# ai-forever/Kandinsky-5

Measured on AMD Instinct MI355X. Metric: DiT denoising steps/sec (2B Lite, 5s 768x512 latent), higher is better.
Workload: dtype bf16

## Files before the change

include/k5.h:

```cpp
#ifndef K5_H
#define K5_H
#include <stdint.h>
#ifdef __cplusplus
extern "C" {
#endif

typedef enum {
  K5_OK = 0, K5_ERR_ARG = 1, K5_ERR_ALIGN = 2, K5_ERR_HIP = 3, K5_ERR_STATE = 4, K5_ERR_KEY = 5,
  K5_ERR_UNSUPPORTED = 6
} k5_status;
typedef enum { K5_F32 = 0, K5_BF16 = 1, K5_F16 = 2 } k5_dtype;
typedef enum { K5_EPI_BIAS = 0, K5_EPI_BIAS_M = 1, K5_EPI_GELU = 2, K5_EPI_GATE = 3, K5_EPI_F32 = 4  } k5_epilogue;

#define K5_ABI_VERSION 11
int k5_abi_version(void);
const char* k5_last_error(void);


int k5_gemm_bf16(const void* A, const void* W, const float* bias, void* C, int M, int N, int K, int lda,
                 int ldw, int ldc, int epilogue, const void* resid, int ldr, const float* gate, void* stream);
int k5_gemm_bf16_variant(const void* A, const void* W, const float* bias, void* C, int M, int N, int K, int lda, int ldw, int ldc,
                         int epilogue, const void* resid, int ldr, const float* gate, void* stream, int kernel, int token_tile);

int k5_gemm_bf16_f32out(const void* A, const void* W, float* C, int M, int N, int K, int lda, int ldw, int ldc,
                        float alpha, int causal_hw, void* stream);

int k5_causal_softmax_bf16(const float* scores, void* P, int S, int hw, int lds, int ldp, void* stream);
int k5_vae_attention512_bf16(const void* q, const void* k, const void* vt, void* o, int S, int hw, int ldqk, int ldvt, int ldo,
                             float scale, void* stream);

int k5_attention_bf16(const void* Q, const void* K, const void* Vt, void* O, int H, int q_len, int kv_len,
                      int ldq, int ldk, int ldvt, int ldo, void* stream);

int64_t k5_attention_state_size(int H, int q_len);
int k5_attention_bf16_range(const void* Q, const void* K, const void* Vt, void* O, int H, int q_len, int kv_len,
                            int ldq, int ldk, int ldvt, int ldo, float score_bound, int tile_off0, int tile_cnt,
                            int tile_skip_at, int tile_skip_n, void* state, int flags, void* stream);
// ... 245 lines not shown
```

kandinsky-5_amd/csrc/engine.hip:

```cpp
#include <math.h>
#include <stdarg.h>
#include <stdio.h>
#include <stdlib.h>
#include <string.h>

#include <map>
#include <optional>
#include <string>
#include <vector>

#include <dlfcn.h>
#include <pthread.h>
#include <rccl/rccl.h>

#include "k5_common.h"
#include "k5_kernels.h"
#include "ipc_comm.h"

static thread_local char g_err[1024] = "";
void k5_set_error(const char* fmt, ...) {
  va_list ap;
  va_start(ap, fmt);
  vsnprintf(g_err, sizeof(g_err), fmt, ap);
  va_end(ap);
// ... 274 lines not shown
  DevBuf ws_attn_bal;
  DevBuf ws_attn_stats, ws_attn_flags, ws_attn_cnt, ws_attn_part;
  long long nabla_possible = 0;
  int nabla_list_rows = 4;
  int attn_mode = 0;
  int sp_pass1_tiles = 0;
  int nabla_group_rows = 0, nabla_grp_now = 4;
  int nabla_pair_frames = 1;
  void* nabla_tap = nullptr; long long nabla_tap_cap = 0, nabla_tap_n = 0;
  int nabla_fuse_means = 1;
  DevBuf ws_nabla_kept;
  unsigned long long* h_nabla_kept = nullptr;
  long long nabla_hint_possible = 0;
  bool nabla_hint_pending = false;
  int sp_nabla_passes = 1;
  int fuse_qnorm = 0;
  int fuse_qnorm_auto = 1;
  bool fuse_now = false, leave_collect = false;
  int fuse_last = -1;
  DevBuf ws_leave_sig;
  DevBuf ws_pref_snap;
  unsigned int* h_leave_sig = nullptr;
  bool row_offsets = true;
  bool anchor = true;
  DevBuf ws_attn_anchor;
  int sp_slices = 1;
  int sp_mode = 0;
  DevBuf ws_u_send, ws_u_recv, ws_u_vsend, ws_u_vrecv, ws_u_o, ws_u_orecv, ws_u_stats;
  hipEvent_t ev_u_o = nullptr, ev_u_back = nullptr;
  DevBuf ws_u_qrecv;
// ... 291 lines not shown
  const bool vis = !strcmp(fam_attn, "attn_self");
  const bool f8_in = vis && sa_fp8_in(d, a, rows);
  const bool f8_out = vis && (d->fp8_mask & 4) && a.wo8.p && rows >= 256;
  if (h8_ready && !f8_in) { k5_set_error("internal: e4m3 activations handed to a bf16 projection"); return K5_ERR_ARG; }
  if (f8_in) {
    K5CHK(d->ws_h8.ensure((size_t)rows * D));
    if (!h8_ready) {
      Scope sc(d, s, "elementwise");
      K5CHK(k5_launch_quant_rows_fp8(h, d->ws_h8.p, nullptr, rows, D, D, D, s));
    }
    Scope sc(d, s, "gemm");
    K5CHK(k5_launch_gemm_fp8(d->ws_h8.p, a.wqk8.p, a.sqk.as<float>(), qk, rows, 2 * D, D, D, D, 2 * D, K5_EPI_BIAS, nullptr, 0, nullptr, s, a.bqk.as<float>(), 0));
    K5CHK(k5_launch_gemm_fp8(a.wv8.p, d->ws_h8.p, a.sv.as<float>(), vt, D, rows, D, D, D, ldvt, K5_EPI_BIAS, nullptr, 0, nullptr, s, a.bv.as<float>(), 1));
  } else {
    Scope sc(d, s, "gemm");
    K5CHK(k5_launch_gemm_bf16(h, a.wqk.p, a.bqk.as<float>(), qk, rows, 2 * D, D, D, D, 2 * D, K5_EPI_BIAS, nullptr, 0, nullptr, s));
    K5CHK(k5_launch_gemm_bf16(a.wv.p, h, a.bv.as<float>(), vt, D, rows, D, D, D, ldvt, K5_EPI_BIAS_M, nullptr, 0, nullptr, s));
  }
  const bool pre = vis && rows % 64 == 0;
  const bool by_data = pre && d->attn_mode == K5_ATTN_AUTO;
  SoftmaxForm sf;
  const bool fuse_q = pre && !nabla && (d->fuse_qnorm || d->fuse_now) && ((by_data && d->row_offsets) || d->attn_mode == K5_ATTN_ONLINE);
  unsigned int* leave_sig = (d->leave_collect && d->ws_leave_sig.p) ? d->ws_leave_sig.as<unsigned int>() : nullptr;
  const bool fuse_means = pre && nabla && nabla_means_fused(d, rows, 2 * H);
  const int grp = pre ? attn_group_rows(d, nabla != nullptr, false) : 4;
  if (by_data) K5CHK(ensure_attn_flags(d, s));
  const K5QueryNorm qn{a.norm.as<float>(), cosT, sinT, by_data ? d->ws_attn_cnt.as<unsigned long long>() : nullptr};
  {
    Scope sc(d, s, "elementwise");
    const int32_t hc[2] = {H, 2 * H};
    void* kc = nullptr;
    void *mq = nullptr, *mk = nullptr;
// ... 1737 lines not shown
    if (value != K5_ATTN_AUTO && value != K5_ATTN_ONLINE) { k5_set_error("attn_mode must be 0 or 1"); return K5_ERR_ARG; }
    d->attn_mode = value; return K5_OK;
  }
  if (!strcmp(name, "sp_pass1_tiles")) { if (value < 0) return K5_ERR_ARG; d->sp_pass1_tiles = value; return K5_OK; }
  if (!strcmp(name, "sp_mode")) { if (value < 0 || value > 2) return K5_ERR_ARG; d->sp_mode = value; d->sp_user_set |= 1; return K5_OK; }
  if (!strcmp(name, "sp_autotune")) { d->sp_autotune = value != 0; if (value > 1) d->sp_tuned = false; return K5_OK; }
  if (!strcmp(name, "attn_row_offsets")) { d->row_offsets = value != 0; return K5_OK; }
  if (!strcmp(name, "attn_anchor")) { d->anchor = value != 0; return K5_OK; }
  if (!strcmp(name, "attn_pref_reset")) return reset_attn_pref(d, nullptr, true);
  if (!strcmp(name, "cross_kv_batched")) { if (value != 0 && value != 1) return K5_ERR_ARG; d->cross_kv_batched = value; return K5_OK; }
  if (!strcmp(name, "nabla_fuse_means")) { if (value < 0 || value > 2) return K5_ERR_ARG; d->nabla_fuse_means = value; return K5_OK; }
  if (!strcmp(name, "fp8_fuse_ln")) { if (value != 0 && value != 1) return K5_ERR_ARG; d->fp8_fuse_ln = value; return K5_OK; }
  if (!strcmp(name, "nabla_pair_frames")) { if (value != 0 && value != 1) return K5_ERR_ARG; d->nabla_pair_frames = value; return K5_OK; }
  if (!strcmp(name, "nabla_group_rows")) { if (value != 0 && value != 1 && value != 2 && value != 4) return K5_ERR_ARG; d->nabla_group_rows = value; return K5_OK; }
  if (!strcmp(name, "sp_nabla_passes")) { if (value < 1 || value > 2) return K5_ERR_ARG; d->sp_nabla_passes = value; d->sp_user_set |= 4; return K5_OK; }
  if (!strcmp(name, "attn_fuse_qnorm")) { if (value < 0 || value > 2) return K5_ERR_ARG; d->fuse_qnorm = value; return K5_OK; }
  if (!strcmp(name, "attn_fuse_qnorm_auto")) { if (value != 0 && value != 1) return K5_ERR_ARG; d->fuse_qnorm_auto = value; return K5_OK; }
  if (!strcmp(name, "sp_slices")) {
    if (value < 1 || value > 4) return K5_ERR_ARG;
    if (value > 1 && d->comm.comm && !d->comm.can_exchange()) { k5_set_error("sp_slices > 1 needs ncclSend / ncclRecv / ncclGroup* in the RCCL library"); return K5_ERR_STATE; }
    d->sp_slices = value; d->sp_user_set |= 2; return K5_OK;
  }
  if (!strcmp(name, "emulate_world")) {
    if (!d->comm.active() || d->comm.world != 1 || value < 1) { k5_set_error("emulate_world needs a world = 1 communicator"); return K5_ERR_STATE; }
    d->sp_world = value; d->emulated = value > 1;
    if (d->emulated) fprintf(stderr, "libk5: emulate_world=%d — timing-only layout, the results of this handle are garbage\n", value);
    return K5_OK;
  }
  k5_set_error("unknown option %s", name);
  return K5_ERR_ARG;
}
extern "C" int k5_dit_get_option(k5_dit* d, const char* name, int* value) {
  if (!d || !name || !value) return K5_ERR_ARG;
  if (!strcmp(name, "attn_mode")) *value = d->attn_mode;
  else if (!strcmp(name, "sp_pass1_tiles")) *value = d->sp_pass1_tiles;
  else if (!strcmp(name, "sp_mode")) *value = d->sp_mode;
  else if (!strcmp(name, "sp_mode_used")) *value = d->sp_mode_used;
  else if (!strcmp(name, "sp_slices")) *value = d->sp_slices;
  else if (!strcmp(name, "attn_row_offsets")) *value = d->row_offsets ? 1 : 0;
  else if (!strcmp(name, "attn_anchor")) *value = d->anchor ? 1 : 0;
  else if (!strcmp(name, "attn_fuse_qnorm")) *value = d->fuse_qnorm;
  else if (!strcmp(name, "attn_fuse_qnorm_auto")) *value = d->fuse_qnorm_auto;
  else if (!strcmp(name, "attn_fuse_qnorm_used")) *value = d->fuse_last;
  else if (!strcmp(name, "sp_nabla_passes")) *value = d->sp_nabla_passes;
  else if (!strcmp(name, "sp_autotune")) *value = d->sp_autotune ? 1 : 0;
  else if (!strcmp(name, "sp_tuned")) *value = d->sp_tuned ? 1 : 0;
  else if (!strcmp(name, "fp8_effective")) {
    int m = d->fp8_mask;
    if (d->comm.active()) { m &= ~4; if (sp_schedule(d, d->last_nabla) != 0) m &= ~2; }
    *value = m;
  }
  else if (!strcmp(name, "rccl_ranks")) {
    *value = 0;
    if (d->comm.comm && d->comm.CommCount) { int n = 0; *value = d->comm.CommCount(d->comm.comm, &n) == ncclSuccess ? n : -1; }
    else if (d->comm.active()) *value = -1;
// ... 104 lines not shown
```

kandinsky-5_amd/csrc/gemm_bf16.hip:

```cpp

#include <type_traits>

#include "k5_common.h"
#include "k5_kernels.h"

namespace {
inline int k5_num_cu() {
  int dev = 0; hipDeviceProp_t prop;
  if (hipGetDevice(&dev) != hipSuccess || hipGetDeviceProperties(&prop, dev) != hipSuccess) return -1;
  return prop.multiProcessorCount > 0 ? prop.multiProcessorCount : 256;
}

constexpr int BM = 128, BN = 128, BK = 64;
constexpr int TILE_BYTES = 128 * 128;

struct GemmP {
  const bf16_t* A; const bf16_t* W; bf16_t* C;
  const float* bias;
  const bf16_t* resid;
  const float* gate;
  int M, N, K, lda, ldw, ldc, ldr;
  int tiles_m, tiles_n;
  float alpha;
  int causal_hw;
// ... 417 lines not shown
    return w * (full + (rem == 0 ? 0.0 : (tail_ok && full > 0 && 2 * rem < num_cu ? 0.3 : 1.0)));
  };
  const bool mt3 = cost(192, 0.75, false) < 0.97 * cost(256, 1.0, true);
  return mt3 ? launch_k8_mt<EPI, 3>(p, stream, num_cu) : launch_k8_mt<EPI, 4>(p, stream, num_cu);
}

constexpr int W4_PAD = 1056, W4_OP = 32 * W4_PAD, W4_STAGE = 2 * W4_OP, W4_LDS = 2 * W4_STAGE;
constexpr int w4_stages(int mt) { return mt == 4 ? 3 : 2; }
constexpr int w4_stage_bytes(int mt) { return mt == 4 ? W4_OP + 16 * W4_PAD : W4_STAGE; }
constexpr int w4_ops_bytes(int mt) { return w4_stages(mt) * w4_stage_bytes(mt); }
static_assert(w4_ops_bytes(4) + 4 * 1024 <= 160 * 1024 && w4_ops_bytes(8) == W4_LDS, "LDS budget of the four-wave kernel");
constexpr int W4_PF_BYTES = 4 * 1024;
constexpr int W4_DMA_AUX = 0;
typedef __attribute__((address_space(3))) void w4_lds_t;

template <int EPI, int MT = 8>
__global__ __launch_bounds__(256) __attribute__((amdgpu_waves_per_eu(1, 1))) void gemm_bf16_w4_kernel(GemmP p) {
  static_assert(MT == 8 || MT == 6 || MT == 4, "token tiles per wave");
  static_assert(EPI != K5_EPI_F32 || MT == 8, "the frame-causal tile walk is written for 256-row tiles");
  constexpr int TM = 32 * MT;
  constexpr int NM = 16 * MT, HM = 8 * MT;
  constexpr int XD = MT == 4 ? 4 : 8;
  constexpr int ND = 8 + XD;
  constexpr int NST = w4_stages(MT), STG = w4_stage_bytes(MT), OPS = NST * STG;
  extern __shared__ __attribute__((aligned(16))) char dsm[];
  const int tid = threadIdx.x, lane = tid & 63, wave = __builtin_amdgcn_readfirstlane(tid >> 6);
  const int wn = wave & 1, wm = wave >> 1;
  const int l15 = lane & 15, lc = lane >> 4;

  const int nblk = p.lid_limit;
  const int xcd = blockIdx.x & 7, slot = blockIdx.x >> 3, per_xcd = (gridDim.x + 7 - xcd) >> 3;
  const int q8 = nblk >> 3, r8 = nblk & 7;
  const int x_first = xcd < r8 ? xcd * (q8 + 1) : r8 * (q8 + 1) + (xcd - r8) * q8, x_cnt = q8 + (xcd < r8 ? 1 : 0);
  constexpr int GM = 4;
  const int per_group = GM * p.tiles_n;
  auto tile_origin = [&](int lid, int& m0, int& n0) {
    if (EPI == K5_EPI_F32 && p.causal_hw > 0) {
      int i = 0;
      for (;; ++i) {
        const int last = min((i + 1) * K8_BM, p.M) - 1;
        const int c = min(p.tiles_n, (min(p.N, (last / p.causal_hw + 1) * p.causal_hw) + K8_BN - 1) / K8_BN);
        if (lid < c || i + 1 >= p.tiles_m) break;
        lid -= c;
      }
      m0 = i * K8_BM; n0 = lid * K8_BN;
      return;
    }
    const int g = lid / per_group, first_m = g * GM;
    const int gsz = min(p.tiles_m - first_m, GM);
    m0 = (first_m + (lid % per_group) % gsz) * TM;
    n0 = ((lid % per_group) / gsz) * K8_BN;
  };
  const int nk = p.K / BK;
  const int ntl = slot < x_cnt ? (x_cnt - slot + per_xcd - 1) / per_xcd : 0;
  if (ntl == 0) return;
  const uint32_t ldw2 = (uint32_t)p.ldw * 2u, lda2 = (uint32_t)p.lda * 2u;
  const uint32_t vw0 = (uint32_t)(16 * (lane >> 3)) * ldw2 + (uint32_t)(lane & 7) * 16u;
  const uint32_t vx0 = (uint32_t)(16 * (lane >> 3)) * lda2 + (uint32_t)(lane & 7) * 16u;
  const int drow = 128 * (wave >> 1) + 8 * (wave & 1);
  const int dslot = 8 * wave;
  const int drow_x = MT == 4 ? 4 * wave : drow, dslot_x = MT == 4 ? 4 * wave : dslot;
  uint32_t vw = vw0, vx = vx0;
  __amdgpu_buffer_rsrc_t rW, rX;
  int d_si = 0, d_cnt = 0;
  auto set_dma_tile = [&](int si) {
    int m0, n0;
    tile_origin(x_first + si * per_xcd + slot, m0, n0);
    const int rows_w = min(p.N - n0, K8_BN), rows_x = min(p.M - m0, MT == 4 ? 128 : K8_BM);
    rW = __builtin_amdgcn_make_buffer_rsrc((void*)(reinterpret_cast<const char*>(p.W) + (size_t)n0 * ldw2), 0,
                                           (int)(((uint32_t)(rows_w - 1) * (uint32_t)p.ldw + (uint32_t)p.K) * 2u), 0x00020000);
    rX = __builtin_amdgcn_make_buffer_rsrc((void*)(reinterpret_cast<const char*>(p.A) + (size_t)m0 * lda2), 0,
                                           (int)(((uint32_t)(rows_x - 1) * (uint32_t)p.lda + (uint32_t)p.K) * 2u), 0x00020000);
    d_cnt = 0; vw = vw0; vx = vx0;
  };
  auto dma_w = [&](int so) {
#pragma unroll
    for (int jj = 0; jj < 8; ++jj)
      __builtin_amdgcn_raw_ptr_buffer_load_lds(rW, (w4_lds_t*)(dsm + so + (dslot + jj) * W4_PAD), 16, vw,
                                               (uint32_t)(drow + jj) * ldw2, 0, W4_DMA_AUX);
  };
  auto dma_x = [&](int so) {
#pragma unroll
    for (int jj = 0; jj < XD; ++jj)
      __builtin_amdgcn_raw_ptr_buffer_load_lds(rX, (w4_lds_t*)(dsm + so + W4_OP + (dslot_x + jj) * W4_PAD), 16, vx,
                                               (uint32_t)(drow_x + jj) * lda2, 0, W4_DMA_AUX);
  };
  auto dma_advance = [&]() {
// ... 94 lines not shown
      const bool wrap = o_cur == STG;
      o_cur = o_cur == 2 * STG ? 0 : o_cur + STG;
      wb_nx = wrap ? wb_nx - 2 * STG : wb_nx + STG;
      xb_nx = wrap ? xb_nx - 2 * STG : xb_nx + STG;
    }
  };

  for (int si = 0; si < ntl; ++si) {
    ktile(std::integral_constant<int, 0>{}, std::true_type{});
    ktile(std::integral_constant<int, 1>{}, std::false_type{});
    for (int t = 1; t < nk / 2; ++t) {
      ktile(std::integral_constant<int, 0>{}, std::false_type{});
      ktile(std::integral_constant<int, 1>{}, std::false_type{});
    }
    asm volatile("s_nop 15\n\ts_nop 15" ::: "memory");
    int m0, n0;
    tile_origin(x_first + si * per_xcd + slot, m0, n0);
    int tid2 = threadIdx.x;
    asm volatile("" : "+v"(tid2));
    const int e_l15 = tid2 & 15, e_lc = (tid2 >> 4) & 3, e_wave = tid2 >> 6;
    const int e_wn = e_wave & 1, e_wm = e_wave >> 1;
    auto epilogue = [&](auto HB) {
      constexpr bool has_bias = decltype(HB)::value;
      const int nb = n0 + 128 * e_wn + 4 * e_lc;
      if constexpr (EPI == K5_EPI_F32) {
        float* cf = reinterpret_cast<float*>(p.C);
#pragma unroll
        for (int j = 0; j < MT; ++j) {
          const int m = m0 + 16 * MT * e_wm + 16 * j + e_l15;
#pragma unroll
          for (int i = 0; i < 8; ++i) {
            const int n = nb + 16 * i;
// ... 7 lines not shown
      }
      f32x4 bvec[8];
      float* vslot = reinterpret_cast<float*>(dsm + OPS + 1024 * e_wave);
      if constexpr (EPI == K5_EPI_GATE) {
        const int l = tid2 & 63;
#pragma unroll
        for (int h = 0; h < 2; ++h) {
          const int c = min(n0 + 128 * e_wn + 2 * l + h, p.N - 1);
          vslot[2 * l + h] = has_bias ? p.bias[c] : 0.f;
          vslot[128 + 2 * l + h] = p.gate[c];
        }
        asm volatile("s_waitcnt vmcnt(0) lgkmcnt(0)" ::: "memory");
      } else {
#pragma unroll
        for (int i = 0; i < 8; ++i) {
          const int nc = min(nb + 16 * i, p.N - 4);
          if (EPI != K5_EPI_BIAS_M && has_bias) bvec[i] = *reinterpret_cast<const f32x4*>(p.bias + nc);
        }
      }
      const uint32_t vaddr = (uint32_t)(uintptr_t)(w4_lds_t*)(dsm + OPS) + 1024u * (uint32_t)e_wave + 16u * (uint32_t)e_lc;
      f32x4 bq[2][2], gq[2][2];
#define W4_VEC_FETCH(IQ, B) do { W4_RD(bq[B][0], vaddr, 128 * (IQ)); W4_RD(bq[B][1], vaddr, 128 * (IQ) + 64); \
                                W4_RD(gq[B][0], vaddr, 512 + 128 * (IQ)); W4_RD(gq[B][1], vaddr, 512 + 128 * (IQ) + 64); } while (0)
      auto finish_rows = [&](int j, float bm, const u32x2 (&rr)[8]) {
        const int m = m0 + 16 * MT * e_wm + 16 * j + e_l15;
        if constexpr (EPI == K5_EPI_GATE) W4_VEC_FETCH(0, 0);
#pragma unroll
        for (int iq = 0; iq < 4; ++iq) {
          if constexpr (EPI == K5_EPI_GATE) {
            if (iq == 0) W4_VEC_FETCH(1, 1);
            if (iq == 1) W4_VEC_FETCH(2, 0);
            if (iq == 2) W4_VEC_FETCH(3, 1);
            if (iq < 3) asm volatile("s_waitcnt lgkmcnt(4)" ::: "memory");
            else asm volatile("s_waitcnt lgkmcnt(0)" ::: "memory");
            __builtin_amdgcn_sched_barrier(0);
            asm volatile("" : "+v"(bq[iq & 1][0]), "+v"(bq[iq & 1][1]), "+v"(gq[iq & 1][0]), "+v"(gq[iq & 1][1]));
          }
          u32x2 o[2];
#pragma unroll
          for (int h = 0; h < 2; ++h) {
            const int i = 2 * iq + h;
            float v[4];
            W4_ACC(v, 8 * j + i);
            f32x4 bv = f32x4{0.f, 0.f, 0.f, 0.f}, gv = bv;
            if constexpr (EPI == K5_EPI_GATE) { bv = bq[iq & 1][h]; gv = gq[iq & 1][h]; }
            else if (EPI != K5_EPI_BIAS_M && has_bias) bv = bvec[i];
#pragma unroll
            for (int e = 0; e < 4; ++e) {
              if (EPI == K5_EPI_BIAS_M) v[e] += bm;
              else if (has_bias) v[e] += bv[e];
              if (EPI == K5_EPI_GELU) v[e] = bf_round(v[e]);
            }
            if (EPI == K5_EPI_GELU) { gelu_erf_x2(v[0], v[1]); gelu_erf_x2(v[2], v[3]); }
            if (EPI == K5_EPI_GATE) {
              v[0] = __uint_as_float(rr[i][0] << 16) + gv[0] * bf_round(v[0]);
              v[1] = __uint_as_float(rr[i][0] & 0xffff0000u) + gv[1] * bf_round(v[1]);
              v[2] = __uint_as_float(rr[i][1] << 16) + gv[2] * bf_round(v[2]);
              v[3] = __uint_as_float(rr[i][1] & 0xffff0000u) + gv[3] * bf_round(v[3]);
            }
            o[h] = u32x2{pack_bf16x2(v[0], v[1]), pack_bf16x2(v[2], v[3])};
          }
#pragma unroll
          for (int d = 0; d < 2; ++d) {
            const auto sw = __builtin_amdgcn_permlane16_swap(o[0][d], o[1][d], false, false);
            o[0][d] = sw[0]; o[1][d] = sw[1];
          }
          const int n = n0 + 128 * e_wn + 16 * (2 * iq + (e_lc & 1)) + 8 * (e_lc >> 1);
          if (m < p.M && n < p.N) *reinterpret_cast<u32x4*>(p.C + (size_t)m * p.ldc + n) = u32x4{o[0][0], o[0][1], o[1][0], o[1][1]};
        }
      };
      if constexpr (EPI == K5_EPI_GATE) {
        u32x2 rr[2][8];
        auto load_rows = [&](int j, u32x2 (&dst)[8]) {
          const int m = min(m0 + 16 * MT * e_wm + 16 * j + e_l15, p.M - 1);
#pragma unroll
          for (int i = 0; i < 8; ++i) dst[i] = *reinterpret_cast<const u32x2*>(p.resid + (size_t)m * p.ldr + min(nb + 16 * i, p.N - 4));
        };
        load_rows(0, rr[0]);
#pragma unroll
        for (int j = 0; j < MT; ++j) {
          if (j + 1 < MT) load_rows(j + 1, rr[(j + 1) & 1]);
          asm volatile("" ::: "memory");
          finish_rows(j, 0.f, rr[j & 1]);
          asm volatile("" ::: "memory");
        }
      } else {
        constexpr int G = MT == 6 ? 3 : 4;
#pragma unroll
        for (int jh = 0; jh < MT / G; ++jh) {
          float bias_m[G];
#pragma unroll
          for (int jj = 0; jj < G; ++jj)
            bias_m[jj] = (EPI == K5_EPI_BIAS_M && has_bias) ? p.bias[min(m0 + 16 * MT * e_wm + 16 * (G * jh + jj) + e_l15, p.M - 1)] : 0.f;
          const u32x2 none[8] = {};
#pragma unroll
          for (int jj = 0; jj < G; ++jj) finish_rows(G * jh + jj, bias_m[jj], none);
          asm volatile("" ::: "memory");
        }
      }
    };
    if (p.bias) epilogue(std::true_type{}); else epilogue(std::false_type{});
    __builtin_amdgcn_s_waitcnt(0x0F70);
  }
#undef W4_VEC_FETCH
#undef W4_XB
#undef W4_MF
#undef W4_MF0
#undef W4_ACC
#undef W4_RD
  asm volatile("s_waitcnt vmcnt(0)" ::: "memory");
}

constexpr int Q4_OP = 16 * W4_PAD, Q4_STAGE = 2 * Q4_OP, Q4_NST = 4, Q4_LDS = Q4_NST * Q4_STAGE;

template <int EPI>
__global__ __launch_bounds__(256) void gemm_bf16_q4_kernel(GemmP p) {
  extern __shared__ __attribute__((aligned(16))) char dsm[];
  const int tid = threadIdx.x, lane = tid & 63, wave = __builtin_amdgcn_readfirstlane(tid >> 6);
  const int wn = wave & 1, wm = wave >> 1, l15 = lane & 15, lc = lane >> 4;
  const int plid = p.tail_base + (int)(blockIdx.x >> 2), q = blockIdx.x & 3;
  const int pg = plid / (4 * p.tiles256_n), pfirst = pg * 4, pgsz = min(p.tiles256_m - pfirst, 4);
  const int m0 = (pfirst + (plid % (4 * p.tiles256_n)) % pgsz) * 256 + 128 * (q >> 1);
  const int n0 = ((plid % (4 * p.tiles256_n)) / pgsz) * 256 + 128 * (q & 1);
  if (m0 >= p.M || n0 >= p.N) return;

// ... 179 lines not shown
      case K5_EPI_GATE: hipLaunchKernelGGL(gemm_bf16_glds_kernel<K5_EPI_GATE>, grid, block, 0, stream, p); break;
      default: return K5_ERR_ARG;
    }
    return hipGetLastError() == hipSuccess ? K5_OK : K5_ERR_HIP;
  }
  switch (epi) {
    case K5_EPI_BIAS: hipLaunchKernelGGL(gemm_bf16_kernel<K5_EPI_BIAS>, grid, block, 0, stream, p); break;
    case K5_EPI_BIAS_M: hipLaunchKernelGGL(gemm_bf16_kernel<K5_EPI_BIAS_M>, grid, block, 0, stream, p); break;
    case K5_EPI_GELU: hipLaunchKernelGGL(gemm_bf16_kernel<K5_EPI_GELU>, grid, block, 0, stream, p); break;
    case K5_EPI_GATE: hipLaunchKernelGGL(gemm_bf16_kernel<K5_EPI_GATE>, grid, block, 0, stream, p); break;
    default: return K5_ERR_ARG;
  }
  return hipGetLastError() == hipSuccess ? K5_OK : K5_ERR_HIP;
}

int k5_launch_gemm_bf16_f32out(const void* A, const void* W, float* C, int M, int N, int K, int lda, int ldw, int ldc,
                               float alpha, int causal_hw, hipStream_t stream) {
  if (M <= 0 || N <= 0 || K <= 0 || causal_hw < 0) return K5_ERR_ARG;
  if ((K & 7) || (lda & 7) || (ldw & 7)) return K5_ERR_ALIGN;
  GemmP p;
  p.A = (const bf16_t*)A; p.W = (const bf16_t*)W; p.C = (bf16_t*)C; p.bias = nullptr; p.resid = nullptr; p.gate = nullptr;
  p.M = M; p.N = N; p.K = K; p.lda = lda; p.ldw = ldw; p.ldc = ldc; p.ldr = 0; p.alpha = alpha; p.lid_limit = 0; p.tail_base = -1; p.tiles256_m = p.tiles256_n = 0;
  p.causal_hw = causal_hw;
  const int tm = (M + K8_BM - 1) / K8_BM, tn = (N + K8_BN - 1) / K8_BN;
  long long kept = 0;
  for (int i = 0; i < tm; ++i) {
    const int last = std::min((i + 1) * K8_BM, M) - 1;
    kept += causal_hw > 0 ? std::min(tn, (int)((std::min((long long)N, ((long long)last / causal_hw + 1) * causal_hw) + K8_BN - 1) / K8_BN)) : tn;
  }
  if ((K % (2 * BK)) == 0 && K >= 4 * BK && M >= 512 && N >= 256 && !(N & 3) && !(ldc & 3) && kept >= 256 && kept < (1ll << 30)) {
// ... 15 lines not shown
```

kandinsky-5_amd/csrc/k5_api.hip:

```cpp
#include "k5_kernels.h"

void k5_set_error(const char* fmt, ...);

static int ret(int st, const char* what) {
  if (st != K5_OK) {
    const hipError_t e = hipGetLastError();
    k5_set_error("%s: status %d (%s)", what, st, e == hipSuccess ? "argument/alignment" : hipGetErrorString(e));
  }
  return st;
}

template <class A>
static A attn_args(const void* Q, const void* K, const void* Vt, void* O, int H, int q_len, int kv_len, int ldq, int ldk, int ldvt, int ldo,
                   void* stream) {
  A a;
  a.Q = Q; a.K = K; a.Vt = Vt; a.O = O;
  a.H = H; a.q_len = q_len; a.kv_len = kv_len; a.ldq = ldq; a.ldk = ldk; a.ldvt = ldvt; a.ldo = ldo;
  a.stream = (hipStream_t)stream;
  return a;
}

extern "C" {

int k5_gemm_bf16(const void* A, const void* W, const float* bias, void* C, int M, int N, int K, int lda, int ldw,
// ... 5 lines not shown
int k5_gemm_bf16_variant(const void* A, const void* W, const float* bias, void* C, int M, int N, int K, int lda, int ldw,
                         int ldc, int epilogue, const void* resid, int ldr, const float* gate, void* stream, int kernel, int token_tile) {
  if (token_tile != 0 && token_tile != 128 && token_tile != 192 && token_tile != 256) return ret(K5_ERR_ARG, "k5_gemm_bf16_variant");
  return ret(k5_launch_gemm_bf16(A, W, bias, C, M, N, K, lda, ldw, ldc, epilogue, resid, ldr, gate, (hipStream_t)stream, kernel, token_tile / 32),
             "k5_gemm_bf16_variant");
}

int k5_causal_softmax_bf16(const float* scores, void* P, int S, int hw, int lds, int ldp, void* stream) {
  if (!scores || !P || lds < S) return K5_ERR_ARG;
  return ret(k5_launch_causal_softmax(scores, P, S, hw, lds, ldp, (hipStream_t)stream), "k5_causal_softmax_bf16");
}

int k5_vae_attention512_bf16(const void* q, const void* k, const void* vt, void* o, int S, int hw, int ldqk, int ldvt, int ldo,
                             float scale, void* stream) {
  return ret(k5_launch_vae_attention512(q, k, vt, o, S, hw, ldqk, ldvt, ldo, scale, (hipStream_t)stream), "k5_vae_attention512_bf16");
}

int k5_gemm_bf16_f32out(const void* A, const void* W, float* C, int M, int N, int K, int lda, int ldw, int ldc, float alpha,
                        int causal_hw, void* stream) {
  return ret(k5_launch_gemm_bf16_f32out(A, W, C, M, N, K, lda, ldw, ldc, alpha, causal_hw, (hipStream_t)stream), "k5_gemm_bf16_f32out");
}

int k5_attention_bf16(const void* Q, const void* K, const void* Vt, void* O, int H, int q_len, int kv_len, int ldq,
                      int ldk, int ldvt, int ldo, void* stream) {
  K5AttnRangeArgs a = attn_args<K5AttnRangeArgs>(Q, K, Vt, O, H, q_len, kv_len, ldq, ldk, ldvt, ldo, stream);
  return ret(k5_launch_attention_bf16_range(a), "k5_attention_bf16");
}

int64_t k5_attention_state_size(int H, int q_len) { return (int64_t)k5_attention_state_bytes(H, q_len); }

// ... 345 lines not shown
```

kandinsky-5_amd/csrc/k5_kernels.h:

```cpp
#pragma once
#include <hip/hip_runtime.h>
#include <stdint.h>

#include "k5.h"

int k5_launch_gemm_bf16(const void* A, const void* W, const float* bias, void* C, int M, int N, int K,
                        int lda, int ldw, int ldc, int epi, const void* resid, int ldr,
                        const float* gate, hipStream_t stream,
                        int force_kernel = 0,
                        int force_mt = 0);

size_t k5_attention_state_bytes(int H, int q_len);
struct K5TileSegments { int len, stride, skip; };
struct K5SparsePass { const int* begin; float* state; int flags; int late_pass; };
struct K5QueryNorm { const float* w; const float* cos; const float* sin; unsigned long long* counters; };
struct K5KeyCentre { const float* centre; const float* radius; const float* row_anchor = nullptr; };
enum { K5_ATTN_AUTO = 0, K5_ATTN_ONLINE = 1 };
struct K5AttnArgs {
  const void* Q = nullptr; const void* K = nullptr; const void* Vt = nullptr; void* O = nullptr;
  int H = 0, q_len = 0, kv_len = 0, ldq = 0, ldk = 0, ldvt = 0, ldo = 0;
  float score_bound = 0.f;
  int vt_chunk_keys = 0; long long vt_chunk_stride = 0;
  hipStream_t stream = nullptr;
  float* balance_ws = nullptr;
  bool k_prescaled = false;
// ... 123 lines not shown
```

kandinsky-5_amd/kandinsky/_engine.py:

```python
from __future__ import annotations

import ctypes as C
import os
from typing import Optional

import torch

_HERE = os.path.dirname(os.path.abspath(__file__))
LIB_PATH = os.environ.get("K5_LIB", os.path.join(os.path.dirname(_HERE), "lib", "libk5.so"))

K5_OK = 0
ABI_VERSION = 11
K5_F32, K5_BF16, K5_F16 = 0, 1, 2
EPI_BIAS, EPI_BIAS_M, EPI_GELU, EPI_GATE = 0, 1, 2, 3

_DT = {torch.float32: K5_F32, torch.bfloat16: K5_BF16, torch.float16: K5_F16}


class DitConfig(C.Structure):
    _fields_ = [("in_visual_dim", C.c_int), ("in_text_dim", C.c_int), ("in_text_dim2", C.c_int),
                ("time_dim", C.c_int), ("out_visual_dim", C.c_int), ("patch_size", C.c_int * 3),
                ("model_dim", C.c_int), ("ff_dim", C.c_int), ("num_text_blocks", C.c_int),
                ("num_visual_blocks", C.c_int), ("axes_dims", C.c_int * 3), ("visual_cond", C.c_int)]

# ... 27 lines not shown


class VaeConfig(C.Structure):
    _fields_ = [("latent_channels", C.c_int), ("out_channels", C.c_int), ("block_out_channels", C.c_int * 4),
                ("layers_per_block", C.c_int), ("norm_num_groups", C.c_int)]


_lib: Optional[C.CDLL] = None

_P, _I, _F, _I64 = C.c_void_p, C.c_int, C.c_float, C.c_int64
SYMBOLS = {
    "k5_abi_version": (_I, []),
    "k5_last_error": (C.c_char_p, []),
    "k5_gemm_bf16": (_I, [_P, _P, _P, _P, _I, _I, _I, _I, _I, _I, _I, _P, _I, _P, _P]),
    "k5_gemm_bf16_variant": (_I, [_P, _P, _P, _P, _I, _I, _I, _I, _I, _I, _I, _P, _I, _P, _P, _I, _I]),
    "k5_gemm_bf16_f32out": (_I, [_P, _P, _P, _I, _I, _I, _I, _I, _I, _F, _I, _P]),
    "k5_causal_softmax_bf16": (_I, [_P, _P, _I, _I, _I, _I, _P]),
    "k5_vae_attention512_bf16": (_I, [_P, _P, _P, _P, _I, _I, _I, _I, _I, _F, _P]),
    "k5_attention_bf16": (_I, [_P, _P, _P, _P, _I, _I, _I, _I, _I, _I, _I, _P]),
    "k5_attention_state_size": (_I64, [_I, _I]),
    "k5_attention_bf16_range": (_I, [_P, _P, _P, _P, _I, _I, _I, _I, _I, _I, _I, _F, _I, _I, _I, _I, _P, _I, _P]),
    "k5_gemm_fp8": (_I, [_P, _P, _P, _P, _I, _I, _I, _I, _I, _I, _I, _P, _I, _P, _P]),
    "k5_quant_rows_fp8": (_I, [_P, _P, _P, _I, _I, _I, _I, _P]),
    "k5_attention_bf16_prescaled": (_I, [_P, _P, _P, _P, _I, _I, _I, _I, _I, _I, _I, _F, _P]),
    "k5_attention_bf16_prescaled_auto": (_I, [_P, _P, _P, _P, _I, _I, _I, _I, _I, _I, _I, _P, _I, _P, _P]),
    "k5_attention_flags": (_I, [_P, _P, _I, _I, _I, _I, _P, _P]),
    "k5_attention_flags_rows": (_I, [_P, _P, _I, _I, _I, _I, _P, _P, _P]),
    "k5_attention_bf16_prescaled_rows": (_I, [_P, _P, _P, _P, _I, _I, _I, _I, _I, _I, _I, _P, _P, _P, _P]),
    "k5_attention_bf16_prescaled_rows_pass": (_I, [_P, _P, _P, _P, _I, _I, _I, _I, _I, _I, _I, _P, _P, _I, _I, _P, _I, _I, _P, _P]),
    "k5_attention_bf16_prescaled_qnorm_pass": (_I, [_P, _P, _P, _P, _I, _I, _I, _I, _I, _I, _I, _P, _P, _P, _P, _P, _I, _I, _P, _I, _I, _P, _P]),
# ... 184 lines not shown
    M, K = a.shape
    N = w.shape[0]
    if out is None:
        out = torch.empty(M, N, dtype=torch.bfloat16, device=a.device)
    if kernel or token_tile:
        check(lib().k5_gemm_bf16_variant(ptr(a), ptr(w), ptr(bias), ptr(out), M, N, K, a.stride(0), w.stride(0), out.stride(0),
                                         epilogue, ptr(resid), 0 if resid is None else resid.stride(0), ptr(gate),
                                         stream_ptr(a.device), int(kernel), int(token_tile)), "k5_gemm_bf16_variant")
        return out
    check(lib().k5_gemm_bf16(ptr(a), ptr(w), ptr(bias), ptr(out), M, N, K, a.stride(0), w.stride(0), out.stride(0),
                             epilogue, ptr(resid), 0 if resid is None else resid.stride(0), ptr(gate),
                             stream_ptr(a.device)), "k5_gemm_bf16")
    return out


def attention(q, k, vt, num_heads, q_len=None, kv_len=None, out=None, score_bound=None):
    _need_cuda(q, k, vt)
    q_len = q.shape[0] if q_len is None else q_len
    kv_len = k.shape[0] if kv_len is None else kv_len
    if out is None:
        out = torch.empty(q_len, num_heads * 64, dtype=torch.bfloat16, device=q.device)
    if score_bound is not None:
        check(lib().k5_attention_bf16_bounded(ptr(q), ptr(k), ptr(vt), ptr(out), num_heads, q_len, kv_len, q.stride(0),
                                              k.stride(0), vt.stride(0), out.stride(0), float(score_bound),
                                              stream_ptr(q.device)), "k5_attention_bf16_bounded")
        return out
    check(lib().k5_attention_bf16(ptr(q), ptr(k), ptr(vt), ptr(out), num_heads, q_len, kv_len, q.stride(0), k.stride(0),
                                  vt.stride(0), out.stride(0), stream_ptr(q.device)), "k5_attention_bf16")
    return out

# ... 113 lines not shown
```

Measured before the change: 1.908.

## Merge QK and V projection GEMMs into one persistent paired-tile launch

Adds a paired GEMM kernel that runs the QK projection and the transposed V projection as one persistent launch over a combined tile space. A small planner picks the token tile size and an optional split tail. The aim is to cut one launch and fill the partial last wave of tiles across both problems. In exchange the epilogue branches per tile on which problem it serves and picks per-problem bias handling, and merging only happens when both GEMMs already qualify for the w4 path.

```diff
diff --git a/include/k5.h b/include/k5.h
--- a/include/k5.h
+++ b/include/k5.h
@@ -21,6 +21,10 @@
                  int ldw, int ldc, int epilogue, const void* resid, int ldr, const float* gate, void* stream);
 int k5_gemm_bf16_variant(const void* A, const void* W, const float* bias, void* C, int M, int N, int K, int lda, int ldw, int ldc,
                          int epilogue, const void* resid, int ldr, const float* gate, void* stream, int kernel, int token_tile);
+
+int k5_gemm_bf16_pair(const void* A0, const void* W0, const float* bias0, void* C0, int M0, int N0, int lda0, int ldw0, int ldc0,
+                      const void* A1, const void* W1, const float* bias1, void* C1, int M1, int N1, int lda1, int ldw1, int ldc1,
+                      int K, void* stream, int merge, int token_tile, int* merged);
 
 int k5_gemm_bf16_f32out(const void* A, const void* W, float* C, int M, int N, int K, int lda, int ldw, int ldc,
                         float alpha, int causal_hw, void* stream);
diff --git a/kandinsky-5_amd/csrc/engine.hip b/kandinsky-5_amd/csrc/engine.hip
--- a/kandinsky-5_amd/csrc/engine.hip
+++ b/kandinsky-5_amd/csrc/engine.hip
@@ -312,6 +312,8 @@
   long long nabla_hint_possible = 0;
   bool nabla_hint_pending = false;
   int sp_nabla_passes = 1;
+  int merge_qkv = 1;
+  unsigned long long merged_qkv_launches = 0;
   int fuse_qnorm = 0;
   int fuse_qnorm_auto = 1;
   bool fuse_now = false, leave_collect = false;
@@ -633,8 +635,10 @@
     K5CHK(k5_launch_gemm_fp8(a.wv8.p, d->ws_h8.p, a.sv.as<float>(), vt, D, rows, D, D, D, ldvt, K5_EPI_BIAS, nullptr, 0, nullptr, s, a.bv.as<float>(), 1));
   } else {
     Scope sc(d, s, "gemm");
-    K5CHK(k5_launch_gemm_bf16(h, a.wqk.p, a.bqk.as<float>(), qk, rows, 2 * D, D, D, D, 2 * D, K5_EPI_BIAS, nullptr, 0, nullptr, s));
-    K5CHK(k5_launch_gemm_bf16(a.wv.p, h, a.bv.as<float>(), vt, D, rows, D, D, D, ldvt, K5_EPI_BIAS_M, nullptr, 0, nullptr, s));
+    const K5GemmProblem gqk{h, a.wqk.p, a.bqk.as<float>(), qk, rows, 2 * D, D, D, 2 * D}, gv{a.wv.p, h, a.bv.as<float>(), vt, D, rows, D, D, ldvt};
+    int merged = 0;
+    K5CHK(k5_launch_gemm_bf16_pair(gqk, gv, D, s, d->merge_qkv ? 1 : 0, 0, &merged));
+    d->merged_qkv_launches += (unsigned long long)merged;
   }
   const bool pre = vis && rows % 64 == 0;
   const bool by_data = pre && d->attn_mode == K5_ATTN_AUTO;
@@ -2402,6 +2406,7 @@
   if (!strcmp(name, "nabla_pair_frames")) { if (value != 0 && value != 1) return K5_ERR_ARG; d->nabla_pair_frames = value; return K5_OK; }
   if (!strcmp(name, "nabla_group_rows")) { if (value != 0 && value != 1 && value != 2 && value != 4) return K5_ERR_ARG; d->nabla_group_rows = value; return K5_OK; }
   if (!strcmp(name, "sp_nabla_passes")) { if (value < 1 || value > 2) return K5_ERR_ARG; d->sp_nabla_passes = value; d->sp_user_set |= 4; return K5_OK; }
+  if (!strcmp(name, "gemm_merge_qkv")) { if (value != 0 && value != 1) return K5_ERR_ARG; d->merge_qkv = value; return K5_OK; }
   if (!strcmp(name, "attn_fuse_qnorm")) { if (value < 0 || value > 2) return K5_ERR_ARG; d->fuse_qnorm = value; return K5_OK; }
   if (!strcmp(name, "attn_fuse_qnorm_auto")) { if (value != 0 && value != 1) return K5_ERR_ARG; d->fuse_qnorm_auto = value; return K5_OK; }
   if (!strcmp(name, "sp_slices")) {
@@ -2427,6 +2432,8 @@
   else if (!strcmp(name, "sp_slices")) *value = d->sp_slices;
   else if (!strcmp(name, "attn_row_offsets")) *value = d->row_offsets ? 1 : 0;
   else if (!strcmp(name, "attn_anchor")) *value = d->anchor ? 1 : 0;
+  else if (!strcmp(name, "gemm_merge_qkv")) *value = d->merge_qkv;
+  else if (!strcmp(name, "gemm_merged_qkv_launches")) *value = (int)(d->merged_qkv_launches & 0x7fffffffull);
   else if (!strcmp(name, "attn_fuse_qnorm")) *value = d->fuse_qnorm;
   else if (!strcmp(name, "attn_fuse_qnorm_auto")) *value = d->fuse_qnorm_auto;
   else if (!strcmp(name, "attn_fuse_qnorm_used")) *value = d->fuse_last;
diff --git a/kandinsky-5_amd/csrc/gemm_bf16.hip b/kandinsky-5_amd/csrc/gemm_bf16.hip
--- a/kandinsky-5_amd/csrc/gemm_bf16.hip
+++ b/kandinsky-5_amd/csrc/gemm_bf16.hip
@@ -3,6 +3,7 @@
 
 #include "k5_common.h"
 #include "k5_kernels.h"
+#include "gemm_pair_tiles.h"
 
 namespace {
 inline int k5_num_cu() {
@@ -455,8 +456,10 @@
 constexpr int W4_DMA_AUX = 0;
 typedef __attribute__((address_space(3))) void w4_lds_t;
 
-template <int EPI, int MT = 8>
-__global__ __launch_bounds__(256) __attribute__((amdgpu_waves_per_eu(1, 1))) void gemm_bf16_w4_kernel(GemmP p) {
+constexpr int W4_EPI_PAIR = 64;
+template <int EPI, int MT>
+K5_DEV void gemm_w4_tiles(const GemmP& p, const GemmP& p1) {
+  constexpr bool PAIR = EPI == W4_EPI_PAIR;
   static_assert(MT == 8 || MT == 6 || MT == 4, "token tiles per wave");
   static_assert(EPI != K5_EPI_F32 || MT == 8, "the frame-causal tile walk is written for 256-row tiles");
   constexpr int TM = 32 * MT;
@@ -475,7 +478,13 @@
   const int x_first = xcd < r8 ? xcd * (q8 + 1) : r8 * (q8 + 1) + (xcd - r8) * q8, x_cnt = q8 + (xcd < r8 ? 1 : 0);
   constexpr int GM = 4;
   const int per_group = GM * p.tiles_n;
-  auto tile_origin = [&](int lid, int& m0, int& n0) {
+  auto tile_origin = [&](int lid, int& m0, int& n0, int& which) {
+    which = 0;
+    if constexpr (PAIR) {
+      const K5PairTile t = k5_pair_tile(lid, p.tail_base, TM, p.tiles_m, p.tiles_n, p1.tiles_m, p1.tiles_n);
+      m0 = t.m0; n0 = t.n0; which = t.problem;
+      return;
+    }
     if (EPI == K5_EPI_F32 && p.causal_hw > 0) {
       int i = 0;
       for (;; ++i) {
@@ -495,9 +504,9 @@
   const int nk = p.K / BK;
   const int ntl = slot < x_cnt ? (x_cnt - slot + per_xcd - 1) / per_xcd : 0;
   if (ntl == 0) return;
-  const uint32_t ldw2 = (uint32_t)p.ldw * 2u, lda2 = (uint32_t)p.lda * 2u;
-  const uint32_t vw0 = (uint32_t)(16 * (lane >> 3)) * ldw2 + (uint32_t)(lane & 7) * 16u;
-  const uint32_t vx0 = (uint32_t)(16 * (lane >> 3)) * lda2 + (uint32_t)(lane & 7) * 16u;
+  uint32_t ldw2 = (uint32_t)p.ldw * 2u, lda2 = (uint32_t)p.lda * 2u;
+  uint32_t vw0 = (uint32_t)(16 * (lane >> 3)) * ldw2 + (uint32_t)(lane & 7) * 16u;
+  uint32_t vx0 = (uint32_t)(16 * (lane >> 3)) * lda2 + (uint32_t)(lane & 7) * 16u;
   const int drow = 128 * (wave >> 1) + 8 * (wave & 1);
   const int dslot = 8 * wave;
   const int drow_x = MT == 4 ? 4 * wave : drow, dslot_x = MT == 4 ? 4 * wave : dslot;
@@ -505,13 +514,26 @@
   __amdgpu_buffer_rsrc_t rW, rX;
   int d_si = 0, d_cnt = 0;
   auto set_dma_tile = [&](int si) {
-    int m0, n0;
-    tile_origin(x_first + si * per_xcd + slot, m0, n0);
-    const int rows_w = min(p.N - n0, K8_BN), rows_x = min(p.M - m0, MT == 4 ? 128 : K8_BM);
-    rW = __builtin_amdgcn_make_buffer_rsrc((void*)(reinterpret_cast<const char*>(p.W) + (size_t)n0 * ldw2), 0,
-                                           (int)(((uint32_t)(rows_w - 1) * (uint32_t)p.ldw + (uint32_t)p.K) * 2u), 0x00020000);
-    rX = __builtin_amdgcn_make_buffer_rsrc((void*)(reinterpret_cast<const char*>(p.A) + (size_t)m0 * lda2), 0,
-                                           (int)(((uint32_t)(rows_x - 1) * (uint32_t)p.lda + (uint32_t)p.K) * 2u), 0x00020000);
+    int m0, n0, which;
+    tile_origin(x_first + si * per_xcd + slot, m0, n0, which);
+    if constexpr (!PAIR) {
+      const int rows_w = min(p.N - n0, K8_BN), rows_x = min(p.M - m0, MT == 4 ? 128 : K8_BM);
+      rW = __builtin_amdgcn_make_buffer_rsrc((void*)(reinterpret_cast<const char*>(p.W) + (size_t)n0 * ldw2), 0,
+                                             (int)(((uint32_t)(rows_w - 1) * (uint32_t)p.ldw + (uint32_t)p.K) * 2u), 0x00020000);
+      rX = __builtin_amdgcn_make_buffer_rsrc((void*)(reinterpret_cast<const char*>(p.A) + (size_t)m0 * lda2), 0,
+                                             (int)(((uint32_t)(rows_x - 1) * (uint32_t)p.lda + (uint32_t)p.K) * 2u), 0x00020000);
+    } else {
+      const GemmP& t = which ? p1 : p;
+      ldw2 = (uint32_t)t.ldw * 2u; lda2 = (uint32_t)t.lda * 2u;
+      vw0 = (uint32_t)(16 * (lane >> 3)) * ldw2 + (uint32_t)(lane & 7) * 16u;
+      vx0 = (uint32_t)(16 * (lane >> 3)) * lda2 + (uint32_t)(lane & 7) * 16u;
+      const int rows_w = min(t.N - n0, K8_BN), rows_x = min(t.M - m0, MT == 4 ? 128 : K8_BM);
+      const int bytes_x = rows_x > 0 ? (int)(((uint32_t)(rows_x - 1) * (uint32_t)t.lda + (uint32_t)p.K) * 2u) : 0;
+      if (rows_x <= 0) m0 = 0;
+      rW = __builtin_amdgcn_make_buffer_rsrc((void*)(reinterpret_cast<const char*>(t.W) + (size_t)n0 * ldw2), 0,
+                                             (int)(((uint32_t)(rows_w - 1) * (uint32_t)t.ldw + (uint32_t)p.K) * 2u), 0x00020000);
+      rX = __builtin_amdgcn_make_buffer_rsrc((void*)(reinterpret_cast<const char*>(t.A) + (size_t)m0 * lda2), 0, bytes_x, 0x00020000);
+    }
     d_cnt = 0; vw = vw0; vx = vx0;
   };
   auto dma_w = [&](int so) {
@@ -636,8 +658,10 @@
       ktile(std::integral_constant<int, 1>{}, std::false_type{});
     }
     asm volatile("s_nop 15\n\ts_nop 15" ::: "memory");
-    int m0, n0;
-    tile_origin(x_first + si * per_xcd + slot, m0, n0);
+    int m0, n0, which;
+    tile_origin(x_first + si * per_xcd + slot, m0, n0, which);
+    int eM = p.M, eN = p.N, eldc = p.ldc; bf16_t* eC = p.C; const float* ebias = p.bias;
+    if constexpr (PAIR) { if (which) { eM = p1.M; eN = p1.N; eldc = p1.ldc; eC = p1.C; ebias = p1.bias; } }
     int tid2 = threadIdx.x;
     asm volatile("" : "+v"(tid2));
     const int e_l15 = tid2 & 15, e_lc = (tid2 >> 4) & 3, e_wave = tid2 >> 6;
@@ -675,8 +699,11 @@
       } else {
 #pragma unroll
         for (int i = 0; i < 8; ++i) {
-          const int nc = min(nb + 16 * i, p.N - 4);
-          if (EPI != K5_EPI_BIAS_M && has_bias) bvec[i] = *reinterpret_cast<const f32x4*>(p.bias + nc);
+          const int nc = min(nb + 16 * i, eN - 4);
+          if constexpr (PAIR) {
+            bvec[i] = f32x4{-0.f, -0.f, -0.f, -0.f};
+            if (!which && ebias) bvec[i] = *reinterpret_cast<const f32x4*>(ebias + nc);
+          } else if (EPI != K5_EPI_BIAS_M && has_bias) bvec[i] = *reinterpret_cast<const f32x4*>(p.bias + nc);
         }
       }
       const uint32_t vaddr = (uint32_t)(uintptr_t)(w4_lds_t*)(dsm + OPS) + 1024u * (uint32_t)e_wave + 16u * (uint32_t)e_lc;
@@ -705,10 +732,11 @@
             W4_ACC(v, 8 * j + i);
             f32x4 bv = f32x4{0.f, 0.f, 0.f, 0.f}, gv = bv;
             if constexpr (EPI == K5_EPI_GATE) { bv = bq[iq & 1][h]; gv = gq[iq & 1][h]; }
-            else if (EPI != K5_EPI_BIAS_M && has_bias) bv = bvec[i];
+            else if (PAIR || (EPI != K5_EPI_BIAS_M && has_bias)) bv = bvec[i];
 #pragma unroll
             for (int e = 0; e < 4; ++e) {
-              if (EPI == K5_EPI_BIAS_M) v[e] += bm;
+              if (PAIR) v[e] = (v[e] + bv[e]) + bm;
+              else if (EPI == K5_EPI_BIAS_M) v[e] += bm;
               else if (has_bias) v[e] += bv[e];
               if (EPI == K5_EPI_GELU) v[e] = bf_round(v[e]);
             }
@@ -727,7 +755,7 @@
             o[0][d] = sw[0]; o[1][d] = sw[1];
           }
           const int n = n0 + 128 * e_wn + 16 * (2 * iq + (e_lc & 1)) + 8 * (e_lc >> 1);
-          if (m < p.M && n < p.N) *reinterpret_cast<u32x4*>(p.C + (size_t)m * p.ldc + n) = u32x4{o[0][0], o[0][1], o[1][0], o[1][1]};
+          if (m < eM && n < eN) *reinterpret_cast<u32x4*>(eC + (size_t)m * eldc + n) = u32x4{o[0][0], o[0][1], o[1][0], o[1][1]};
         }
       };
       if constexpr (EPI == K5_EPI_GATE) {
@@ -752,7 +780,8 @@
           float bias_m[G];
 #pragma unroll
           for (int jj = 0; jj < G; ++jj)
-            bias_m[jj] = (EPI == K5_EPI_BIAS_M && has_bias) ? p.bias[min(m0 + 16 * MT * e_wm + 16 * (G * jh + jj) + e_l15, p.M - 1)] : 0.f;
+            if constexpr (PAIR) bias_m[jj] = (which && ebias) ? ebias[max(min(m0 + 16 * MT * e_wm + 16 * (G * jh + jj) + e_l15, eM - 1), 0)] : -0.f;
+            else bias_m[jj] = (EPI == K5_EPI_BIAS_M && has_bias) ? p.bias[min(m0 + 16 * MT * e_wm + 16 * (G * jh + jj) + e_l15, p.M - 1)] : 0.f;
           const u32x2 none[8] = {};
 #pragma unroll
           for (int jj = 0; jj < G; ++jj) finish_rows(G * jh + jj, bias_m[jj], none);
@@ -760,7 +789,7 @@
         }
       }
     };
-    if (p.bias) epilogue(std::true_type{}); else epilogue(std::false_type{});
+    if (PAIR || p.bias) epilogue(std::true_type{}); else epilogue(std::false_type{});
     __builtin_amdgcn_s_waitcnt(0x0F70);
   }
 #undef W4_VEC_FETCH
@@ -770,6 +799,15 @@
 #undef W4_ACC
 #undef W4_RD
   asm volatile("s_waitcnt vmcnt(0)" ::: "memory");
+}
+
+template <int EPI, int MT = 8>
+__global__ __launch_bounds__(256) __attribute__((amdgpu_waves_per_eu(1, 1))) void gemm_bf16_w4_kernel(GemmP p) {
+  gemm_w4_tiles<EPI, MT>(p, p);
+}
+template <int MT>
+__global__ __launch_bounds__(256) __attribute__((amdgpu_waves_per_eu(1, 1))) void gemm_bf16_w4pair_kernel(GemmP p, GemmP p1) {
+  gemm_w4_tiles<W4_EPI_PAIR, MT>(p, p1);
 }
 
 constexpr int Q4_OP = 16 * W4_PAD, Q4_STAGE = 2 * Q4_OP, Q4_NST = 4, Q4_LDS = Q4_NST * Q4_STAGE;
@@ -979,6 +1017,64 @@
   return hipGetLastError() == hipSuccess ? K5_OK : K5_ERR_HIP;
 }
 
+namespace {
+template <int MT>
+int launch_w4pair_mt(const GemmP& p, const GemmP& p1, int grid, hipStream_t stream) {
+  static const hipError_t attr_rc = hipFuncSetAttribute((const void*)gemm_bf16_w4pair_kernel<MT>, hipFuncAttributeMaxDynamicSharedMemorySize, w4_ops_bytes(MT) + W4_PF_BYTES);
+  if (attr_rc != hipSuccess) return K5_ERR_HIP;
+  hipLaunchKernelGGL((gemm_bf16_w4pair_kernel<MT>), dim3(grid), dim3(256), w4_ops_bytes(MT) + W4_PF_BYTES, stream, p, p1);
+  return hipGetLastError() == hipSuccess ? K5_OK : K5_ERR_HIP;
+}
+}
+
+int k5_launch_gemm_bf16_pair(const K5GemmProblem& g0, const K5GemmProblem& g1, int K, hipStream_t stream, int merge, int force_mt, int* merged) {
+  if (merged) *merged = 0;
+  if (merge < 0 || merge > 2) return K5_ERR_ARG;
+  if (force_mt != 0 && force_mt != 4 && force_mt != 6 && force_mt != 8) return K5_ERR_ARG;
+  static const int num_cu = k5_num_cu();
+  if (num_cu <= 0) return K5_ERR_HIP;
+  auto w4_ok = [&](const K5GemmProblem& g) {
+    return g.M >= 512 && g.N >= 128 && !(g.N & 7) && !(g.ldc & 7) && !(g.lda & 7) && !(g.ldw & 7) && g.A && g.W && g.C &&
+           (long long)g.M * g.lda < (1ll << 30) && (long long)g.N * g.ldw < (1ll << 30);
+  };
+  auto alone_w4 = [&](const K5GemmProblem& g) {
+    const int mt = w4_pick_mt(g.M, g.N, num_cu, 0);
+    return (long long)((g.M + 32 * mt - 1) / (32 * mt)) * ((g.N + 255) / 256) >= W4_MIN_TILES;
+  };
+  bool ok = merge > 0 && K > 0 && (K % (2 * BK)) == 0 && K >= 4 * BK && w4_ok(g0) && w4_ok(g1);
+  if (ok && merge == 1) ok = alone_w4(g0) && alone_w4(g1);
+  if (!ok) {
+    const int rc = k5_launch_gemm_bf16(g0.A, g0.W, g0.bias, g0.C, g0.M, g0.N, K, g0.lda, g0.ldw, g0.ldc, K5_EPI_BIAS, nullptr, 0, nullptr, stream, 0, force_mt);
+    if (rc != K5_OK) return rc;
+    return k5_launch_gemm_bf16(g1.A, g1.W, g1.bias, g1.C, g1.M, g1.N, K, g1.lda, g1.ldw, g1.ldc, K5_EPI_BIAS_M, nullptr, 0, nullptr, stream, 0, force_mt);
+  }
+  const K5PairPlan pl = k5_pair_plan(g0.M, g0.N, g1.M, g1.N, num_cu, force_mt);
+  GemmP p[2];
+  const K5GemmProblem* g[2] = {&g0, &g1};
+  for (int i = 0; i < 2; ++i) {
+    p[i].A = (const bf16_t*)g[i]->A; p[i].W = (const bf16_t*)g[i]->W; p[i].C = (bf16_t*)g[i]->C; p[i].bias = g[i]->bias;
+    p[i].resid = nullptr; p[i].gate = nullptr;
+    p[i].M = g[i]->M; p[i].N = g[i]->N; p[i].K = K; p[i].lda = g[i]->lda; p[i].ldw = g[i]->ldw; p[i].ldc = g[i]->ldc; p[i].ldr = 0;
+    p[i].tiles_m = pl.tiles_m[i]; p[i].tiles_n = pl.tiles_n[i];
+    p[i].alpha = 1.f; p[i].causal_hw = 0; p[i].lid_limit = pl.persistent; p[i].tail_base = -1; p[i].tiles256_m = pl.tiles_m[i]; p[i].tiles256_n = pl.tiles_n[i];
+  }
+  const int grid = std::min(pl.persistent, num_cu);
+  int rc;
+  switch (pl.mt) {
+    case 4: rc = launch_w4pair_mt<4>(p[0], p[1], grid, stream); break;
+    case 6: rc = launch_w4pair_mt<6>(p[0], p[1], grid, stream); break;
+    default: rc = launch_w4pair_mt<8>(p[0], p[1], grid, stream); break;
+  }
+  if (rc != K5_OK) return rc;
+  if (pl.tail_tiles > 0) {
+    p[0].tail_base = pl.persistent; p[0].lid_limit = 2 * pl.tail_tiles;
+    rc = launch_w4pair_mt<4>(p[0], p[1], 2 * pl.tail_tiles, stream);
+    if (rc != K5_OK) return rc;
+  }
+  if (merged) *merged = 1;
+  return K5_OK;
+}
+
 int k5_launch_gemm_bf16_f32out(const void* A, const void* W, float* C, int M, int N, int K, int lda, int ldw, int ldc,
                                float alpha, int causal_hw, hipStream_t stream) {
   if (M <= 0 || N <= 0 || K <= 0 || causal_hw < 0) return K5_ERR_ARG;
diff --git a/kandinsky-5_amd/csrc/gemm_pair_tiles.h b/kandinsky-5_amd/csrc/gemm_pair_tiles.h
--- /dev/null
+++ b/kandinsky-5_amd/csrc/gemm_pair_tiles.h
@@ -0,0 +1,70 @@
+#pragma once
+
+#if defined(__HIPCC__) || defined(__CUDACC__)
+#define K5_PAIR_HD __host__ __device__ inline
+#else
+#define K5_PAIR_HD inline
+#endif
+
+struct K5PairTile { int problem, m0, n0; };
+
+struct K5PairPlan {
+  int mt;
+  int tiles_m[2], tiles_n[2];
+  int tiles;
+  int persistent;
+  int tail_tiles;
+};
+
+K5_PAIR_HD void k5_pair_origin1(int lid, int tiles_m, int tiles_n, int tm, int& m0, int& n0) {
+  const int per_group = 4 * tiles_n;
+  const int g = lid / per_group, first_m = g * 4;
+  const int left = tiles_m - first_m, gsz = left < 4 ? left : 4;
+  m0 = (first_m + (lid % per_group) % gsz) * tm;
+  n0 = ((lid % per_group) / gsz) * 256;
+}
+
+K5_PAIR_HD K5PairTile k5_pair_tile(int entry, int tail_base, int tm, int tiles_m0, int tiles_n0, int tiles_m1, int tiles_n1) {
+  K5PairTile t;
+  int lid = tail_base < 0 ? entry : tail_base + (entry >> 1);
+  const int t0 = tiles_m0 * tiles_n0;
+  t.problem = lid >= t0 ? 1 : 0;
+  if (t.problem) lid -= t0;
+  k5_pair_origin1(lid, t.problem ? tiles_m1 : tiles_m0, t.problem ? tiles_n1 : tiles_n0, tail_base < 0 ? tm : 256, t.m0, t.n0);
+  if (tail_base >= 0) t.m0 += 128 * (entry & 1);
+  return t;
+}
+
+inline K5PairPlan k5_pair_plan(int M0, int N0, int M1, int N1, int num_cu, int force_mt) {
+  const double rel[3] = {1.0, 0.85, 0.63};
+  const int mts[3] = {8, 6, 4};
+  K5PairPlan best{};
+  double best_cost = 1e30;
+  for (int v = 0; v < 3; ++v) {
+    K5PairPlan pl{};
+    pl.mt = mts[v];
+    const int tm = 32 * pl.mt;
+    pl.tiles_m[0] = (M0 + tm - 1) / tm; pl.tiles_n[0] = (N0 + 255) / 256;
+    pl.tiles_m[1] = (M1 + tm - 1) / tm; pl.tiles_n[1] = (N1 + 255) / 256;
+    pl.tiles = pl.tiles_m[0] * pl.tiles_n[0] + pl.tiles_m[1] * pl.tiles_n[1];
+    const int full = pl.tiles / num_cu, rem = pl.tiles % num_cu;
+    const bool split = pl.mt == 8 && full > 0 && rem > 0 && 2 * rem < num_cu;
+    pl.persistent = split ? full * num_cu : pl.tiles;
+    pl.tail_tiles = split ? rem : 0;
+    double c = rel[v] * (full + (rem == 0 ? 0.0 : (split ? 0.85 : 1.0)));
+    if (force_mt == pl.mt) c = -1.0;
+    if (c < best_cost - 1e-9) { best_cost = c; best = pl; }
+  }
+  return best;
+}
+
+struct K5PairWalk { int first, per_xcd, count; };
+K5_PAIR_HD K5PairWalk k5_pair_walk(int block, int grid, int entries) {
+  const int xcd = block & 7, slot = block >> 3, per_xcd = (grid + 7 - xcd) >> 3;
+  const int q8 = entries >> 3, r8 = entries & 7;
+  const int x_first = xcd < r8 ? xcd * (q8 + 1) : r8 * (q8 + 1) + (xcd - r8) * q8, x_cnt = q8 + (xcd < r8 ? 1 : 0);
+  K5PairWalk w;
+  w.first = x_first + slot; w.per_xcd = per_xcd;
+  w.count = slot < x_cnt ? (x_cnt - slot + per_xcd - 1) / per_xcd : 0;
+  return w;
+}
diff --git a/kandinsky-5_amd/csrc/k5_api.hip b/kandinsky-5_amd/csrc/k5_api.hip
--- a/kandinsky-5_amd/csrc/k5_api.hip
+++ b/kandinsky-5_amd/csrc/k5_api.hip
@@ -43,6 +43,15 @@
 int k5_vae_attention512_bf16(const void* q, const void* k, const void* vt, void* o, int S, int hw, int ldqk, int ldvt, int ldo,
                              float scale, void* stream) {
   return ret(k5_launch_vae_attention512(q, k, vt, o, S, hw, ldqk, ldvt, ldo, scale, (hipStream_t)stream), "k5_vae_attention512_bf16");
+}
+
+int k5_gemm_bf16_pair(const void* A0, const void* W0, const float* bias0, void* C0, int M0, int N0, int lda0, int ldw0, int ldc0,
+                      const void* A1, const void* W1, const float* bias1, void* C1, int M1, int N1, int lda1, int ldw1, int ldc1,
+                      int K, void* stream, int merge, int token_tile, int* merged) {
+  if (token_tile != 0 && token_tile != 128 && token_tile != 192 && token_tile != 256) return ret(K5_ERR_ARG, "k5_gemm_bf16_pair");
+  if (M0 <= 0 || N0 <= 0 || M1 <= 0 || N1 <= 0 || K <= 0) return ret(K5_ERR_ARG, "k5_gemm_bf16_pair");
+  const K5GemmProblem g0{A0, W0, bias0, C0, M0, N0, lda0, ldw0, ldc0}, g1{A1, W1, bias1, C1, M1, N1, lda1, ldw1, ldc1};
+  return ret(k5_launch_gemm_bf16_pair(g0, g1, K, (hipStream_t)stream, merge, token_tile / 32, merged), "k5_gemm_bf16_pair");
 }
 
 int k5_gemm_bf16_f32out(const void* A, const void* W, float* C, int M, int N, int K, int lda, int ldw, int ldc, float alpha,
diff --git a/kandinsky-5_amd/csrc/k5_kernels.h b/kandinsky-5_amd/csrc/k5_kernels.h
--- a/kandinsky-5_amd/csrc/k5_kernels.h
+++ b/kandinsky-5_amd/csrc/k5_kernels.h
@@ -9,6 +9,10 @@
                         const float* gate, hipStream_t stream,
                         int force_kernel = 0,
                         int force_mt = 0);
+
+struct K5GemmProblem { const void* A; const void* W; const float* bias; void* C; int M, N, lda, ldw, ldc; };
+int k5_launch_gemm_bf16_pair(const K5GemmProblem& g0, const K5GemmProblem& g1, int K, hipStream_t stream, int merge = 1, int force_mt = 0,
+                             int* merged = nullptr);
 
 size_t k5_attention_state_bytes(int H, int q_len);
 struct K5TileSegments { int len, stride, skip; };
diff --git a/kandinsky-5_amd/kandinsky/_engine.py b/kandinsky-5_amd/kandinsky/_engine.py
--- a/kandinsky-5_amd/kandinsky/_engine.py
+++ b/kandinsky-5_amd/kandinsky/_engine.py
@@ -65,6 +65,7 @@
     "k5_last_error": (C.c_char_p, []),
     "k5_gemm_bf16": (_I, [_P, _P, _P, _P, _I, _I, _I, _I, _I, _I, _I, _P, _I, _P, _P]),
     "k5_gemm_bf16_variant": (_I, [_P, _P, _P, _P, _I, _I, _I, _I, _I, _I, _I, _P, _I, _P, _P, _I, _I]),
+    "k5_gemm_bf16_pair": (_I, [_P, _P, _P, _P, _I, _I, _I, _I, _I, _P, _P, _P, _P, _I, _I, _I, _I, _I, _I, _P, _I, _I, _P]),
     "k5_gemm_bf16_f32out": (_I, [_P, _P, _P, _I, _I, _I, _I, _I, _I, _F, _I, _P]),
     "k5_causal_softmax_bf16": (_I, [_P, _P, _I, _I, _I, _I, _P]),
     "k5_vae_attention512_bf16": (_I, [_P, _P, _P, _P, _I, _I, _I, _I, _I, _F, _P]),
@@ -279,6 +280,15 @@
     return out
 
 
+def gemm_pair(a0, w0, bias0, out0, a1, w1, bias1, out1, merge=1, token_tile=0):
+    _need_cuda(a0, w0, bias0, out0, a1, w1, bias1, out1)
+    merged = C.c_int(0)
+    check(lib().k5_gemm_bf16_pair(ptr(a0), ptr(w0), ptr(bias0), ptr(out0), a0.shape[0], w0.shape[0], a0.stride(0), w0.stride(0), out0.stride(0),
+                                  ptr(a1), ptr(w1), ptr(bias1), ptr(out1), a1.shape[0], w1.shape[0], a1.stride(0), w1.stride(0), out1.stride(0),
+                                  a0.shape[1], stream_ptr(a0.device), int(merge), int(token_tile), C.byref(merged)), "k5_gemm_bf16_pair")
+    return bool(merged.value)
+
+
 def attention(q, k, vt, num_heads, q_len=None, kv_len=None, out=None, score_bound=None):
     _need_cuda(q, k, vt)
     q_len = q.shape[0] if q_len is None else q_len
```

Result: no change. 1.901 (-0.4%).
